# DichenZhang1/libultrahdr_dev

Hardware: AMD Instinct MI355X
Metric: MPixels/sec gain-map generate+apply, 4K P010 batch (higher is better)
Workload: dtype u8/u16 in, f32+f64 math, u8/u32 out

## Files before the change

libultrahdr_dev_amd/csrc/uhdr_kernels.hip:

```cpp
#include "uhdr_kernels.h"

#include <hip/hip_runtime.h>

#include <algorithm>
#include <cmath>

#include "uhdr_apply_px.h"
#include "uhdr_device_math.h"
#include "uhdr_wave_scan.h"

namespace uhdr {

__constant__ float c_idw4[4 * 64];

__constant__ float c_idw4p[64];

hipError_t upload_idw4(const float* tables) {
  float p[64];
  for (int oy = 0; oy < 4; ++oy)
    for (int pr = 0; pr < 2; ++pr)
      for (int k = 0; k < 4; ++k)
        for (int h = 0; h < 2; ++h) p[((oy * 2 + pr) * 4 + k) * 2 + h] = tables[oy * 16 + (2 * pr + h) * 4 + k];
  hipError_t e = hipMemcpyToSymbol(HIP_SYMBOL(c_idw4p), p, sizeof(p));
  if (e != hipSuccess) return e;
  return hipMemcpyToSymbol(HIP_SYMBOL(c_idw4), tables, sizeof(float) * 4 * 64);
}

constexpr float k876 = 1 / 876.0f;
constexpr float k896 = 1 / 896.0f;

constexpr float kP3YR = 0.299f, kP3YG = 0.587f, kP3YB = 0.114f;
constexpr float kP3Cb = 1.772f, kP3Cr = 1.402f;
constexpr float kP3GCb = kP3YB * kP3Cb / kP3YG;
constexpr float kP3GCr = kP3YR * kP3Cr / kP3YG;

typedef float f2 __attribute__((ext_vector_type(2)));
__device__ __forceinline__ f2 pk_fma(f2 a, f2 b, f2 c) { return __builtin_elementwise_fma(a, b, c); }
__device__ __forceinline__ f2 splat(float v) { return (f2){v, v}; }
__device__ __forceinline__ f2 bc_lo(f2 v) { return __builtin_shufflevector(v, v, 0, 0); }
__device__ __forceinline__ f2 bc_hi(f2 v) { return __builtin_shufflevector(v, v, 1, 1); }

__device__ __forceinline__ f2 pk_add_sat(f2 a, f2 b) {
  f2 r;
  asm("v_pk_add_f32 %0, %1, %2 clamp" : "=v"(r) : "v"(a), "v"(b));
  return r;
}
__device__ __forceinline__ f2 pk_mul_sat(f2 a, f2 b) {
  f2 r;
  asm("v_pk_mul_f32 %0, %1, %2 clamp" : "=v"(r) : "v"(a), "v"(b));
  return r;
}
__device__ __forceinline__ f2 pk_fma_sat(f2 a, f2 b, f2 c) {
  f2 r;
  asm("v_pk_fma_f32 %0, %1, %2, %3 clamp" : "=v"(r) : "v"(a), "v"(b), "v"(c));
  return r;
}

template <int HI>
__device__ __forceinline__ f2 pk_fma_sat_bc(f2 a, f2 b, f2 c) {
  f2 r;
  if (HI) asm("v_pk_fma_f32 %0, %1, %2, %3 op_sel:[0,0,1] op_sel_hi:[1,1,1] clamp" : "=v"(r) : "v"(a), "v"(b), "v"(c));
  else asm("v_pk_fma_f32 %0, %1, %2, %3 op_sel_hi:[1,1,0] clamp" : "=v"(r) : "v"(a), "v"(b), "v"(c));
  return r;
}


__device__ __attribute__((noinline)) uint32_t lut_index_wild(float t) {
  const double pos = (double)t + 0.5;
  uint32_t v = 0u;
  if (__builtin_fabs(pos) < 9223372036854775808.0) v = (uint32_t)(long long)pos;
  return v;
}
__device__ __forceinline__ uint32_t round_half_up(float t) {
  int r;
  asm("v_cvt_rpi_i32_f32 %0, %1" : "=v"(r) : "v"(t));
  return (uint32_t)r;
}
__device__ __forceinline__ uint32_t lut_index(float e, uint32_t n) {
  const float t = e * (float)(n - 1u);
  uint32_t v;
  if (__builtin_expect(__float_as_uint(t) < 0x4F000000u, 1)) v = round_half_up(t);
  else v = lut_index_wild(t);
  return min(v, n - 1u);
}
__device__ __forceinline__ uint32_t lut_index_unit(float e, uint32_t n) {
  return round_half_up(e * (float)(n - 1u));
}
__device__ __forceinline__ float gain_lut_entry(uint32_t idx, double log2_min, double log2_max, float boost_factor) {
  const float value = (float)idx / (float)(kGainLutN - 1u);
  const float log_boost = (float)(log2_min * (double)(1.0f - value) + log2_max * (double)value);
  return (float)exp2((double)(log_boost * boost_factor));
}

__global__ void __launch_bounds__(256) k_build_luts(float* lut) {
  const uint32_t i = blockIdx.x * 256u + threadIdx.x;
  if (i >= kLutTotal) return;
  float y;
  if (i < kLutHlgInv) y = srgb_inv_oetf_exact((float)(i - kLutSrgbInv) / (float)(kLutSrgbInvN - 1u));
  else if (i < kLutPqInv) y = hlg_inv_oetf_exact((float)(i - kLutHlgInv) / (float)(kLutHlgInvN - 1u));
  else if (i < kLutHlg) y = pq_inv_oetf_exact((float)(i - kLutPqInv) / (float)(kLutPqInvN - 1u));
  else if (i < kLutPq) y = hlg_oetf_exact((float)(i - kLutHlg) / (float)(kLutHlgN - 1u));
  else y = pq_oetf_exact((float)(i - kLutPq) / (float)(kLutPqN - 1u));
  lut[i] = y;
}
hipError_t launch_build_luts(float* lut, hipStream_t s) {
  hipLaunchKernelGGL(k_build_luts, dim3((kLutTotal + 255u) / 256u), dim3(256), 0, s, lut);
  return hipGetLastError();
}
__global__ void __launch_bounds__(256) k_build_lut_codes(float* lut) {
  const uint32_t i = blockIdx.x * 256u + threadIdx.x;
  const uint32_t t = i >> 16, k = i & 0xFFFFu;
  uint16_t* codes = reinterpret_cast<uint16_t*>(lut + (t ? kCodePq : kCodeHlg));
  codes[k] = (uint16_t)(0x3ffu & (uint32_t)(lut[(t ? kLutPq : kLutHlg) + k] * 1023.0f));
}
hipError_t launch_build_lut_codes(float* lut, hipStream_t s) {
  hipLaunchKernelGGL(k_build_lut_codes, dim3(2u * 65536u / 256u), dim3(256), 0, s, lut);
  return hipGetLastError();
}
__global__ void __launch_bounds__(256) k_build_gain_lut(float* table, double log2_min, double log2_max, float boost_factor) {
  const uint32_t i = blockIdx.x * 256u + threadIdx.x;
  if (i < kGainLutN) table[i] = gain_lut_entry(i, log2_min, log2_max, boost_factor);
}
hipError_t launch_build_gain_lut(float* table, double log2_min, double log2_max, float boost_factor, hipStream_t s) {
  hipLaunchKernelGGL(k_build_gain_lut, dim3(kGainLutN / 256u), dim3(256), 0, s, table, log2_min, log2_max, boost_factor);
  return hipGetLastError();
}


template <int TF>
__device__ __forceinline__ float hdr_inv_oetf(float e) {
  if (TF == 1) return hlg_inv_oetf_guarded(e);
  if (TF == 2) return pq_inv_oetf_guarded(e);
  return e;
}

__device__ __forceinline__ float cvt_word0(uint32_t w) {
  float r;
  asm("v_cvt_f32_u32_sdwa %0, %1 dst_sel:DWORD dst_unused:UNUSED_PAD src0_sel:WORD_0" : "=v"(r) : "v"(w));
  return r;
}
__device__ __forceinline__ float cvt_word1(uint32_t w) {
  float r;
  asm("v_cvt_f32_u32_sdwa %0, %1 dst_sel:DWORD dst_unused:UNUSED_PAD src0_sel:WORD_1" : "=v"(r) : "v"(w));
  return r;
}


constexpr int kGenWhole = 0, kGenFront = 1, kGenBack = 2, kGenLinear = 3, kGenBackLinear = 4;
struct GenMid { f2 r, g, b, hr, hg, hb; };
template <int TF, bool LUT, bool FILTER, bool DEFER = false, int PART = kGenWhole>
__device__ __forceinline__ uint32_t gen_pair(const GenConsts& c, const uint32_t (&hy)[2][4][2],
                                             const uint32_t (&huv)[2][2][2], const uint32_t (&y8)[2][4],
                                             const uint32_t (&u8)[2][2], const uint32_t (&v8)[2][2],
                                             uint8_t (&out)[2], float (&gain)[2], const float* s_srgb, const float* s_hdr,
                                             GenMid* mid = nullptr) {
  f2 r, g, b, hr, hg, hb;
  if (PART == kGenBack || PART == kGenBackLinear) {
    r = mid->r; g = mid->g; b = mid->b; hr = mid->hr; hg = mid->hg; hb = mid->hb;
  } else {
  f2 sy = splat(0.0f), su = splat(0.0f), sv = splat(0.0f);
  f2 hsy = splat(0.0f), hsu = splat(0.0f), hsv = splat(0.0f);
#pragma unroll
  for (int r = 0; r < 2; ++r) {
    f2 uf[2], vf[2], huf[2], hvf[2];
#pragma unroll
    for (int k = 0; k < 2; ++k) {
      const f2 ub = (f2){(float)((u8[0][r] >> (8 * k)) & 0xffu), (float)((u8[1][r] >> (8 * k)) & 0xffu)};
      const f2 vb = (f2){(float)((v8[0][r] >> (8 * k)) & 0xffu), (float)((v8[1][r] >> (8 * k)) & 0xffu)};
      uf[k] = pk_fma(ub, splat(k255), splat(-128.0f * k255));
      vf[k] = pk_fma(vb, splat(k255), splat(-128.0f * k255));
      const uint32_t m0 = huv[0][r][k] & 0xFFC0FFC0u, m1 = huv[1][r][k] & 0xFFC0FFC0u;
      const f2 hu = (f2){cvt_word0(m0), cvt_word0(m1)};
      const f2 hv = (f2){cvt_word1(m0), cvt_word1(m1)};
      huf[k] = pk_fma(hu, splat(k896 * 0.015625f), splat(-64.0f * k896)) - splat(0.5f);
      hvf[k] = pk_fma(hv, splat(k896 * 0.015625f), splat(-64.0f * k896)) - splat(0.5f);
    }
#pragma unroll
    for (int d = 0; d < 2; ++d) {
      const int dy = 2 * r + d;
#pragma unroll
      for (int dx = 0; dx < 4; ++dx) {
        const f2 yb = (f2){(float)((y8[0][dy] >> (8 * dx)) & 0xffu), (float)((y8[1][dy] >> (8 * dx)) & 0xffu)};
        sy += yb * splat(k255);
        su += uf[dx >> 1];
        sv += vf[dx >> 1];
        const uint32_t w0 = hy[0][dy][dx >> 1] & 0xFFC0FFC0u, w1 = hy[1][dy][dx >> 1] & 0xFFC0FFC0u;
        const f2 hb = (dx & 1) ? (f2){cvt_word1(w0), cvt_word1(w1)} : (f2){cvt_word0(w0), cvt_word0(w1)};
        hsy += pk_fma(hb, splat(k876 * 0.015625f), splat(-64.0f * k876));
        hsu += huf[dx >> 1];
        hsv += hvf[dx >> 1];
      }
    }
  }
  sy *= splat(0.0625f); su *= splat(0.0625f); sv *= splat(0.0625f);
  hsy *= splat(0.0625f); hsu *= splat(0.0625f); hsv *= splat(0.0625f);

  r = pk_add_sat(sy, splat(c.sdr_cr) * sv);
  g = pk_add_sat(sy - splat(c.sdr_gcb) * su, -(splat(c.sdr_gcr) * sv));
  b = pk_add_sat(sy, splat(c.sdr_cb) * su);
  hr = pk_add_sat(hsy, splat(c.hdr_cr) * hsv);
  hg = pk_add_sat(hsy - splat(c.hdr_gcb) * hsu, -(splat(c.hdr_gcr) * hsv));
  hb = pk_add_sat(hsy, splat(c.hdr_cb) * hsu);
  }
  static_assert((PART != kGenLinear && PART != kGenBackLinear) || (!LUT && !FILTER), "kGenLinear is the exact path's");
  if (PART != kGenBack && PART != kGenLinear && PART != kGenBackLinear && mid != nullptr) { mid->r = r; mid->g = g; mid->b = b; mid->hr = hr; mid->hg = hg; mid->hb = hb; }
  if (PART == kGenFront) return 0u;

  if (FILTER && !LUT) {
    const f2 fr = (f2){srgb_inv_oetf_fast(r.x), srgb_inv_oetf_fast(r.y)};
    const f2 fg = (f2){srgb_inv_oetf_fast(g.x), srgb_inv_oetf_fast(g.y)};
    const f2 fb = (f2){srgb_inv_oetf_fast(b.x), srgb_inv_oetf_fast(b.y)};
    const f2 fs = (splat(c.lum_r) * fr + splat(c.lum_g) * fg + splat(c.lum_b) * fb) * splat(203.0f);
    f2 qr = hr, qg = hg, qb = hb;
    if (TF == 1) {
      qr = (f2){hlg_inv_oetf_fast(hr.x), hlg_inv_oetf_fast(hr.y)};
      qg = (f2){hlg_inv_oetf_fast(hg.x), hlg_inv_oetf_fast(hg.y)};
      qb = (f2){hlg_inv_oetf_fast(hb.x), hlg_inv_oetf_fast(hb.y)};
    } else if (TF == 2) {
      qr = (f2){pq_inv_oetf_fast(hr.x), pq_inv_oetf_fast(hr.y)};
      qg = (f2){pq_inv_oetf_fast(hg.x), pq_inv_oetf_fast(hg.y)};
      qb = (f2){pq_inv_oetf_fast(hb.x), pq_inv_oetf_fast(hb.y)};
    }
    if (!c.gm_identity) {
      const f2 t0 = splat(c.gm[0]) * qr + splat(c.gm[1]) * qg + splat(c.gm[2]) * qb;
      const f2 t1 = splat(c.gm[3]) * qr + splat(c.gm[4]) * qg + splat(c.gm[5]) * qb;
      const f2 t2 = splat(c.gm[6]) * qr + splat(c.gm[7]) * qg + splat(c.gm[8]) * qb;
      qr = t0; qg = t1; qb = t2;
    }
    const f2 fh = (splat(c.lum_r) * qr + splat(c.lum_g) * qg + splat(c.lum_b) * qb) * splat(c.hdr_white_nits);
    uint32_t fbyte[2], fexact = 0u, doubt = 0u;
    float fgain[2];
#pragma unroll
    for (int k = 0; k < 2; ++k) {
      const float ys = k ? fs.y : fs.x, yh = k ? fh.y : fh.x;
      const float gf = (ys > 0.0f) ? yh * __builtin_amdgcn_rcpf(ys) : 1.0f;
      const float gc = __builtin_amdgcn_fmed3f(gf, c.min_boost, c.max_boost);
      const float v = (__builtin_amdgcn_logf(gc) - c.log2_min) * c.flt_scale;
      const float fl = __builtin_floorf(v), fr2 = v - fl;
      const bool lo = gf < c.flt_lo, hi = gf > c.flt_hi;
      const bool mid = (fr2 >= c.flt_delta) && (fr2 <= 1.0f - c.flt_delta);
      const bool sane = !(ys > 0.0f && ys < 1e-10f) && !(yh != 0.0f && __builtin_fabsf(yh) < 1e-10f);
      if (!((lo || hi || mid) && sane)) doubt |= 1u << k;
      fbyte[k] = lo ? c.enc_byte_min : hi ? c.enc_byte_max : (uint32_t)fl;
      fgain[k] = gf;
      if (!(ys > 0.0f)) fexact |= 1u << k;
    }
    if (DEFER || __builtin_amdgcn_ballot_w64(doubt != 0u) == 0ull) {
      out[0] = (uint8_t)fbyte[0]; out[1] = (uint8_t)fbyte[1];
      gain[0] = fgain[0]; gain[1] = fgain[1];
      return fexact | (doubt << 2);
    }
  }
  constexpr int kLockstep = 6;
  if (LUT) {
    r = (f2){s_srgb[lut_index_unit(r.x, kLutSrgbInvN)], s_srgb[lut_index_unit(r.y, kLutSrgbInvN)]};
    g = (f2){s_srgb[lut_index_unit(g.x, kLutSrgbInvN)], s_srgb[lut_index_unit(g.y, kLutSrgbInvN)]};
    b = (f2){s_srgb[lut_index_unit(b.x, kLutSrgbInvN)], s_srgb[lut_index_unit(b.y, kLutSrgbInvN)]};
  } else {
    float ch[6] = {r.x, r.y, g.x, g.y, b.x, b.y};
#pragma unroll
    for (int i = 0; i < 6; i += kLockstep) {
      float part[kLockstep];
#pragma unroll
      for (int j = 0; j < kLockstep; ++j) part[j] = ch[i + j];
      srgb_inv_oetf_guarded_n<kLockstep>(part);
#pragma unroll
      for (int j = 0; j < kLockstep; ++j) ch[i + j] = part[j];
    }
    r = (f2){ch[0], ch[1]}; g = (f2){ch[2], ch[3]}; b = (f2){ch[4], ch[5]};
  }
  const f2 sdr_nits = (splat(c.lum_r) * r + splat(c.lum_g) * g + splat(c.lum_b) * b) * splat(203.0f);

  if (TF != 0 && LUT) {
    hr = (f2){s_hdr[lut_index_unit(hr.x, kLutHlgInvN)], s_hdr[lut_index_unit(hr.y, kLutHlgInvN)]};
    hg = (f2){s_hdr[lut_index_unit(hg.x, kLutHlgInvN)], s_hdr[lut_index_unit(hg.y, kLutHlgInvN)]};
    hb = (f2){s_hdr[lut_index_unit(hb.x, kLutHlgInvN)], s_hdr[lut_index_unit(hb.y, kLutHlgInvN)]};
  } else if (TF != 0) {
    float ch[6] = {hr.x, hr.y, hg.x, hg.y, hb.x, hb.y};
#pragma unroll
    for (int i = 0; i < 6; i += kLockstep) {
      float part[kLockstep];
#pragma unroll
      for (int j = 0; j < kLockstep; ++j) part[j] = ch[i + j];
      if (TF == 1) hlg_inv_oetf_guarded_n<kLockstep>(part);
      else pq_inv_oetf_guarded_n<kLockstep>(part);
#pragma unroll
      for (int j = 0; j < kLockstep; ++j) ch[i + j] = part[j];
    }
    hr = (f2){ch[0], ch[1]}; hg = (f2){ch[2], ch[3]}; hb = (f2){ch[4], ch[5]};
  }
  if (!c.gm_identity) {
    const f2 t0 = splat(c.gm[0]) * hr + splat(c.gm[1]) * hg + splat(c.gm[2]) * hb;
    const f2 t1 = splat(c.gm[3]) * hr + splat(c.gm[4]) * hg + splat(c.gm[5]) * hb;
    const f2 t2 = splat(c.gm[6]) * hr + splat(c.gm[7]) * hg + splat(c.gm[8]) * hb;
    hr = t0; hg = t1; hb = t2;
  }
  if (PART == kGenLinear || PART == kGenBackLinear) { mid->r = r; mid->g = g; mid->b = b; mid->hr = hr; mid->hg = hg; mid->hb = hb; return 0u; }
  const f2 hdr_nits = (splat(c.lum_r) * hr + splat(c.lum_g) * hg + splat(c.lum_b) * hb) * splat(c.hdr_white_nits);

  gain[0] = raw_gain(sdr_nits.x, hdr_nits.x);
  gain[1] = raw_gain(sdr_nits.y, hdr_nits.y);
#pragma unroll
  for (int k = 0; k < 2; ++k)
    out[k] = encode_gain_guarded(gain[k], c.min_boost, c.max_boost, c.log2_min, c.log2_max, c.enc_scale, c.enc_byte_min,
                                 c.enc_byte_max);
  return 3u;
}

typedef uint32_t u32x4 __attribute__((ext_vector_type(4)));
typedef uint32_t u32x2 __attribute__((ext_vector_type(2)));
__device__ __forceinline__ uint4 ld_stream(const uint4* p) {
  const u32x4 v = __builtin_nontemporal_load(reinterpret_cast<const u32x4*>(p));
  return make_uint4(v.x, v.y, v.z, v.w);
}
__device__ __forceinline__ uint2 ld_stream(const uint2* p) {
  const u32x2 v = __builtin_nontemporal_load(reinterpret_cast<const u32x2*>(p));
  return make_uint2(v.x, v.y);
}
__device__ __forceinline__ uint32_t ld_stream(const uint32_t* p) {
  return __builtin_nontemporal_load(p);
}
__device__ __forceinline__ void st_stream(uint4* p, uint4 v) {
  __builtin_nontemporal_store((u32x4){v.x, v.y, v.z, v.w}, reinterpret_cast<u32x4*>(p));
}
__device__ __forceinline__ void st_stream(uint2* p, uint2 v) {
  __builtin_nontemporal_store((u32x2){v.x, v.y}, reinterpret_cast<u32x2*>(p));
}
__device__ __forceinline__ uint32_t ld8(const uint8_t* p) { return *p; }
__device__ __forceinline__ uint32_t ld16(const uint16_t* p) { return *p; }


template <bool ALIGNED>
__device__ __forceinline__ void load_pair(const GenConsts& c, const GenImage& im, const uint8_t* im_v, uint32_t my, uint32_t pr,
                                          bool two, uint32_t (&hy)[2][4][2], uint32_t (&huv)[2][2][2], uint32_t (&y8)[2][4],
                                          uint32_t (&u8)[2][2], uint32_t (&v8)[2][2]) {
  const uint32_t mx = pr * 2u;
  if (ALIGNED) {
    const uint32_t hoff = 4u * my * im.hy_stride + 8u * pr, yoff = 4u * my * im.y_stride + 8u * pr;
#pragma unroll
    for (int r = 0; r < 4; ++r) {
      const uint4 q = ld_stream(reinterpret_cast<const uint4*>(im.hy + (hoff + r * im.hy_stride)));
      hy[0][r][0] = q.x; hy[0][r][1] = q.y; hy[1][r][0] = q.z; hy[1][r][1] = q.w;
      const uint2 p = ld_stream(reinterpret_cast<const uint2*>(im.y + (yoff + r * im.y_stride)));
      y8[0][r] = p.x; y8[1][r] = p.y;
    }
    const uint32_t huvoff = 2u * my * im.huv_stride + 8u * pr, coff = 2u * my * im.c_stride + 4u * pr;
#pragma unroll
    for (int r = 0; r < 2; ++r) {
      const uint4 q = ld_stream(reinterpret_cast<const uint4*>(im.huv + (huvoff + r * im.huv_stride)));
      huv[0][r][0] = q.x; huv[0][r][1] = q.y; huv[1][r][0] = q.z; huv[1][r][1] = q.w;
      const uint32_t uu = ld_stream(reinterpret_cast<const uint32_t*>(im.u + (coff + r * im.c_stride)));
      const uint32_t vv = ld_stream(reinterpret_cast<const uint32_t*>(im_v + (coff + r * im.c_stride)));
      u8[0][r] = uu & 0xffffu; u8[1][r] = uu >> 16;
      v8[0][r] = vv & 0xffffu; v8[1][r] = vv >> 16;
    }
  } else {
#pragma unroll
    for (int k = 0; k < 2; ++k) {
      const bool on = (k == 0) || two;
      const uint32_t x0 = 4u * (mx + k);
#pragma unroll
      for (int r = 0; r < 4; ++r) {
        const uint16_t* hrow = im.hy + (size_t)(4u * my + r) * im.hy_stride + x0;
        const uint8_t* yrow = im.y + (size_t)(4u * my + r) * im.y_stride + x0;
        hy[k][r][0] = on ? (ld16(hrow) | (ld16(hrow + 1) << 16)) : 0u;
        hy[k][r][1] = on ? (ld16(hrow + 2) | (ld16(hrow + 3) << 16)) : 0u;
        y8[k][r] = on ? (ld8(yrow) | (ld8(yrow + 1) << 8) | (ld8(yrow + 2) << 16) | (ld8(yrow + 3) << 24)) : 0u;
      }
#pragma unroll
      for (int r = 0; r < 2; ++r) {
        const uint16_t* crow = im.huv + (size_t)(2u * my + r) * im.huv_stride + x0;
        const uint8_t* urow = im.u + (size_t)(2u * my + r) * im.c_stride + (x0 >> 1);
        const uint8_t* vrow = im_v + (size_t)(2u * my + r) * im.c_stride + (x0 >> 1);
        huv[k][r][0] = on ? (ld16(crow) | (ld16(crow + 1) << 16)) : 0u;
        huv[k][r][1] = on ? (ld16(crow + 2) | (ld16(crow + 3) << 16)) : 0u;
        u8[k][r] = on ? (ld8(urow) | (ld8(urow + 1) << 8)) : 0u;
        v8[k][r] = on ? (ld8(vrow) | (ld8(vrow + 1) << 8)) : 0u;
      }
    }
  }
}

template <int CTRL, int ROWS>
__device__ __forceinline__ float dpp_move(float v) {
  return __int_as_float(__builtin_amdgcn_update_dpp(__float_as_int(v), __float_as_int(v), CTRL, ROWS, 0xF, false));
}
template <bool MAX>
__device__ __forceinline__ float wave_extreme(float v) {
#define UHDR_EXT(CTRL, ROWS) v = MAX ? fmaxf(v, dpp_move<CTRL, ROWS>(v)) : fminf(v, dpp_move<CTRL, ROWS>(v))
  UHDR_EXT(0xB1, 0xF);
  UHDR_EXT(0x4E, 0xF);
  UHDR_EXT(0x141, 0xF);
  UHDR_EXT(0x140, 0xF);
  UHDR_EXT(0x142, 0xA);
  UHDR_EXT(0x143, 0xC);
#undef UHDR_EXT
  return __int_as_float(__builtin_amdgcn_readlane(__float_as_int(v), 63));
}
__device__ __forceinline__ void wave_minmax(float& vmin, float& vmax) {
  vmin = wave_extreme<false>(vmin);
  vmax = wave_extreme<true>(vmax);
}
__device__ __forceinline__ void publish_minmax(float gmin, float gmax, uint32_t* keys) {
  if ((threadIdx.x & 63u) == 0u && gmin <= gmax) {
    const uint32_t kmin = ~float_to_key(gmin), kmax = float_to_key(gmax);
    if (__hip_atomic_load(&keys[0], __ATOMIC_RELAXED, __HIP_MEMORY_SCOPE_AGENT) < kmin) atomicMax(&keys[0], kmin);
    if (__hip_atomic_load(&keys[1], __ATOMIC_RELAXED, __HIP_MEMORY_SCOPE_AGENT) < kmax) atomicMax(&keys[1], kmax);
  }
}

template <int TF, bool ALIGNED, bool LUT>
__device__ __forceinline__ void exact_pair(const GenConsts& c, const GenImage& im, const uint8_t* im_v, uint32_t my,
                                           uint32_t pr, bool two, const float* s_srgb, const float* s_hdr, uint8_t (&o)[2], float (&gn)[2]) {
  uint32_t hy[2][4][2], huv[2][2][2], y8[2][4], u8[2][2], v8[2][2];
  load_pair<ALIGNED>(c, im, im_v, my, pr, two, hy, huv, y8, u8, v8);
  gen_pair<TF, LUT, false>(c, hy, huv, y8, u8, v8, o, gn, s_srgb, s_hdr);
}


template <int TF, bool ALIGNED, bool LUT, bool FILTER, int TILES, bool DEFER, int BLOCK = kGenBlock>
__global__ void __launch_bounds__(BLOCK, 1) k_generate(const GenConsts c, const GenBatch b) {
  __shared__ float s_srgb[LUT ? kLutSrgbInvN : 1];
  __shared__ float s_hdr[(LUT && TF != 0) ? kLutHlgInvN : 1];
  __shared__ float s_kept[(FILTER && DEFER) ? TILES * 2 * BLOCK : 1];
  if (LUT) {
    for (uint32_t i = threadIdx.x; i < kLutSrgbInvN / 4u; i += BLOCK)
      reinterpret_cast<float4*>(s_srgb)[i] = reinterpret_cast<const float4*>(c.lut + kLutSrgbInv)[i];
    if (TF != 0) {
      const float4* src = reinterpret_cast<const float4*>(c.lut + (TF == 1 ? kLutHlgInv : kLutPqInv));
      for (uint32_t i = threadIdx.x; i < kLutHlgInvN / 4u; i += BLOCK) reinterpret_cast<float4*>(s_hdr)[i] = src[i];
    }
    __syncthreads();
  }
  const uint32_t img_i = blockIdx.x, blk = blockIdx.y;
  const GenImage& im = b.img[img_i];
  const uint8_t* im_v = im.u + (size_t)im.c_stride * (c.height / 2u);
  const uint32_t pairs_per_row = (c.map_w + 1u) >> 1;
  const uint32_t total = pairs_per_row * c.map_h;
  const bool stats = c.stat_keys != nullptr;
  float emin = __builtin_inff(), emax = -__builtin_inff();
  float amin = __builtin_inff(), amax = -__builtin_inff();
  uint32_t kept_exact = 0u, kept_valid = 0u, kept_doubt = 0u;
  uint32_t n_saved = 0u;
  uint32_t* wslot = (FILTER && DEFER && c.stat_slots != 0u)
                        ? c.stat_ws + (size_t)kStatWords * blockIdx.x + kStatHdr + (blockIdx.y * (uint32_t)(BLOCK / 64) + (threadIdx.x >> 6)) * kStatSlotWords
                        : nullptr;

#pragma unroll 1
  for (uint32_t t = 0; t < (uint32_t)TILES; ++t) {
    const uint32_t idx = (blk * (uint32_t)TILES + t) * (uint32_t)BLOCK + threadIdx.x;
    if (idx >= total) break;
    const uint32_t my = idx / pairs_per_row;
    const uint32_t pr = idx - my * pairs_per_row;
    const uint32_t mx = pr * 2u;
    const bool two = ALIGNED || (mx + 1u < c.map_w);

    uint32_t hy[2][4][2], huv[2][2][2], y8[2][4], u8[2][2], v8[2][2];
    load_pair<ALIGNED>(c, im, im_v, my, pr, two, hy, huv, y8, u8, v8);

    uint8_t o[2];
    float gn[2];
    GenMid mid;
    const uint32_t ex = gen_pair<TF, LUT, FILTER, DEFER>(c, hy, huv, y8, u8, v8, o, gn, s_srgb, s_hdr, (FILTER && DEFER) ? &mid : nullptr);
    const uint8_t o0 = o[0], o1 = o[1];
    if (FILTER && DEFER) {
      uint32_t dm = (ex >> 2) & (two ? 3u : 1u);
      if (c.stat_slots != 0u) {
        const unsigned long long dmask = __builtin_amdgcn_ballot_w64(dm != 0u);
        if (dmask != 0ull) {
          const uint32_t pos = n_saved + (uint32_t)__builtin_popcountll(dmask & ((1ull << (threadIdx.x & 63u)) - 1ull));
          n_saved += (uint32_t)__builtin_popcountll(dmask);
          if (dm != 0u && pos < kStatSlotSaved) {
            float4* e = reinterpret_cast<float4*>(wslot + 16u + pos * 16u);
            e[0] = make_float4(__uint_as_float((idx << 3) | dm), mid.r.x, mid.r.y, mid.g.x);
            e[1] = make_float4(mid.g.y, mid.b.x, mid.b.y, mid.hr.x);
            e[2] = make_float4(mid.hr.y, mid.hg.x, mid.hg.y, mid.hb.x);
            e[3] = make_float4(mid.hb.y, 0.0f, 0.0f, 0.0f);
            dm = 0u;
          }
        }
      }
      kept_doubt |= dm << (2u * t);
      if (stats) {
        s_kept[(2u * t) * BLOCK + threadIdx.x] = gn[0];
        s_kept[(2u * t + 1u) * BLOCK + threadIdx.x] = gn[1];
        const uint32_t valid = (two ? 3u : 1u) & ~((ex >> 2) & 3u);
        kept_exact |= (ex & 3u) << (2u * t);
        kept_valid |= valid << (2u * t);
        if (valid & 1u) { amin = fminf(amin, gn[0]); amax = fmaxf(amax, gn[0]); }
        if (valid & 2u) { amin = fminf(amin, gn[1]); amax = fmaxf(amax, gn[1]); }
        if (ex & valid & 1u) { emin = fminf(emin, gn[0]); emax = fmaxf(emax, gn[0]); }
        if (ex & valid & 2u) { emin = fminf(emin, gn[1]); emax = fmaxf(emax, gn[1]); }
      }
    } else {
      emin = fminf(emin, gn[0]); emax = fmaxf(emax, gn[0]);
      if (two) { emin = fminf(emin, gn[1]); emax = fmaxf(emax, gn[1]); }
    }
    uint8_t* mp = im.map + (size_t)my * c.map_w + mx;
    if (ALIGNED) {
      *reinterpret_cast<uint16_t*>(mp) = (uint16_t)(o0 | ((uint32_t)o1 << 8));
    } else {
      mp[0] = o0;
      if (two) mp[1] = o1;
    }
  }
  if (FILTER && !DEFER) return;
  if (!FILTER && !stats) return;
  uint32_t* keys = stats ? c.stat_keys + (size_t)c.stat_stride * img_i : nullptr;

  if (FILTER) {
    uint32_t* ws = c.stat_ws + (size_t)kStatWords * img_i;
    uint32_t cand = 0u;
    if (stats) {
      wave_minmax(amin, amax);
      float wmin = emin, wmax = emax;
      wave_minmax(wmin, wmax);
      const float e = c.flt_gain_rel;
      uint32_t* est = c.stat_spread != 0u ? ws + kStatEst + 2u * (blk % kStatLists) : ws;
      uint32_t e0 = __hip_atomic_load(&est[0], __ATOMIC_RELAXED, __HIP_MEMORY_SCOPE_AGENT);
      uint32_t e1 = __hip_atomic_load(&est[1], __ATOMIC_RELAXED, __HIP_MEMORY_SCOPE_AGENT);
      const uint32_t k0 = __hip_atomic_load(&keys[0], __ATOMIC_RELAXED, __HIP_MEMORY_SCOPE_AGENT);
      const uint32_t k1 = __hip_atomic_load(&keys[1], __ATOMIC_RELAXED, __HIP_MEMORY_SCOPE_AGENT);
      if (amin <= amax) {
        const uint32_t m0 = ~float_to_key(amin), m1 = float_to_key(amax);
        if ((threadIdx.x & 63u) == 0u) {
          if (e0 < m0) atomicMax(&est[0], m0);
          if (e1 < m1) atomicMax(&est[1], m1);
        }
        e0 = e0 < m0 ? m0 : e0; e1 = e1 < m1 ? m1 : e1;
      }
      float min_hi = fminf(k1 != 0u ? key_to_float(~k0) : __builtin_inff(), wmin);
      float max_lo = fmaxf(k1 != 0u ? key_to_float(k1) : -__builtin_inff(), wmax);
      if (e1 != 0u) {
        const float pmin = key_to_float(~e0), pmax = key_to_float(e1);
        min_hi = fminf(min_hi, pmin + e * __builtin_fabsf(pmin));
        max_lo = fmaxf(max_lo, pmax - e * __builtin_fabsf(pmax));
      }
#pragma unroll
      for (uint32_t t = 0; t < (uint32_t)TILES; ++t)
#pragma unroll
        for (uint32_t k = 0; k < 2u; ++k) {
          const uint32_t bit = 1u << (2u * t + k);
          if ((kept_valid & bit) && !(kept_exact & bit)) {
            const float a = s_kept[(2u * t + k) * BLOCK + threadIdx.x], slack = e * __builtin_fabsf(a);
            if ((a - slack <= min_hi) || (a + slack >= max_lo)) cand |= 1u << t;
          }
        }
    }
    unsigned long long mask[TILES];
    uint32_t total = 0u;
#pragma unroll
    for (uint32_t t = 0; t < (uint32_t)TILES; ++t) {
      mask[t] = __builtin_amdgcn_ballot_w64((((kept_doubt >> (2u * t)) & 3u) | ((cand >> t) & 1u)) != 0u);
      total += (uint32_t)__builtin_popcountll(mask[t]);
    }
    if (total != 0u || c.stat_slots != 0u) {
      const uint32_t lane = threadIdx.x & 63u, list = blk % kStatLists;
      uint32_t base = 0u, cap = kStatCap;
      uint32_t* lw = ws + kStatHdr + list * kStatCap;
      if (c.stat_slots != 0u) {
        lw = wslot;
        const bool over = total > kStatSlotPlain;
        const uint32_t ns = n_saved < kStatSlotSaved ? n_saved : kStatSlotSaved;
        if (lane == 0u) {
          ws[kStatSlotCnt + blk * (uint32_t)(BLOCK / 64) + (threadIdx.x >> 6)] = over ? 0u : (total | (ns << 8));
          if (over) __hip_atomic_store(&ws[6], 1u, __ATOMIC_RELAXED, __HIP_MEMORY_SCOPE_AGENT);
        }
        ++lw;
        cap = over ? 0u : kStatSlotPlain;
      } else {
        if (lane == 0u) base = atomicAdd(&ws[8u + list], total);
        base = (uint32_t)__builtin_amdgcn_readfirstlane((int)base);
      }
#pragma unroll
      for (uint32_t t = 0; t < (uint32_t)TILES; ++t) {
        const uint32_t flags = ((kept_doubt >> (2u * t)) & 3u) | (((cand >> t) & 1u) << 2);
        const uint32_t pos = base + (uint32_t)__builtin_popcountll(mask[t] & ((1ull << lane) - 1ull));
        if (flags != 0u && pos < cap) lw[pos] = (((blk * (uint32_t)TILES + t) * (uint32_t)BLOCK + threadIdx.x) << 3) | flags;
        base += (uint32_t)__builtin_popcountll(mask[t]);
      }
    }
    if (!stats) return;
  }
  wave_minmax(emin, emax);
  publish_minmax(emin, emax, keys);
}

__global__ void k_stats_finalize(uint32_t* keys, int n) {
  const int i = blockIdx.x * blockDim.x + threadIdx.x;
  if (i >= n) return;
  const uint32_t k0 = keys[2 * i], k1 = keys[2 * i + 1];
  float mn = __builtin_inff(), mx = -__builtin_inff();
  if (k1 != 0u) { mn = key_to_float(~k0); mx = key_to_float(k1); }
  keys[2 * i] = __float_as_uint(mn);
  keys[2 * i + 1] = __float_as_uint(mx);
}

static_assert(kStatLists == 64u, "k_generate_resolve reads the list counts with one wave");
template <int TF, bool ALIGNED>
__global__ void __launch_bounds__(256) k_generate_resolve(const GenConsts c, const GenBatch b) {
  const uint32_t img_i = blockIdx.x;
  const GenImage& im = b.img[img_i];
  const uint8_t* im_v = im.u + (size_t)im.c_stride * (c.height / 2u);
  uint32_t* ws = c.stat_ws + (size_t)kStatWords * img_i;
  const uint32_t pairs_per_row = (c.map_w + 1u) >> 1, total = pairs_per_row * c.map_h;
  const bool stats = c.stat_out != nullptr;
  float emin = __builtin_inff(), emax = -__builtin_inff();
  __shared__ uint32_t s_first[kStatSlotWaves + 1u];
  __shared__ uint8_t s_ns[kStatSlotWaves];
  __shared__ uint32_t s_sweep;
  const bool slots = c.stat_slots != 0u;
  if (slots) {
    static_assert(kStatSlotWaves == 4u * 256u, "four waves' counts per thread");
    __shared__ uint32_t s_part[4];
    uint32_t n4[4];
    const uint4 cw4 = *reinterpret_cast<const uint4*>(ws + kStatSlotCnt + 4u * threadIdx.x);
    const uint32_t cws[4] = {cw4.x, cw4.y, cw4.z, cw4.w};
#pragma unroll
    for (uint32_t j = 0; j < 4u; ++j) {
      const uint32_t w = 4u * threadIdx.x + j;
      const uint32_t cw = w < c.stat_slots ? cws[j] : 0u;
      s_ns[w] = (uint8_t)(cw >> 8);
      n4[j] = (cw & 0xFFu) + (cw >> 8);
    }
    const uint32_t over = __hip_atomic_load(&ws[6], __ATOMIC_RELAXED, __HIP_MEMORY_SCOPE_AGENT);
    const uint32_t mine = n4[0] + n4[1] + n4[2] + n4[3];
    const uint32_t before = block_exclusive_sum<256>(mine, s_part);
    s_first[4u * threadIdx.x] = before;
    s_first[4u * threadIdx.x + 1u] = before + n4[0];
    s_first[4u * threadIdx.x + 2u] = before + n4[0] + n4[1];
    s_first[4u * threadIdx.x + 3u] = before + n4[0] + n4[1] + n4[2];
    if (threadIdx.x == 255u) { s_first[kStatSlotWaves] = before + mine; s_sweep = over; }
  } else if (threadIdx.x < 64u) {
    const uint32_t cnt = ws[8u + threadIdx.x];
    const bool over = __builtin_amdgcn_ballot_w64(cnt > kStatCap) != 0ull;
    uint32_t inc = min(cnt, kStatCap);
#pragma unroll
    for (int off = 1; off < 64; off <<= 1) {
      const uint32_t v = (uint32_t)__shfl_up((int)inc, off, 64);
      if ((int)threadIdx.x >= off) inc += v;
    }
    s_first[threadIdx.x + 1u] = inc;
    if (threadIdx.x == 0) { s_first[0] = 0u; s_sweep = over ? 1u : 0u; }
  }
  __syncthreads();
  const bool sweep = s_sweep != 0u;
  const uint32_t nl = slots ? kStatSlotWaves : kStatLists;
  const uint32_t n = sweep ? total : s_first[nl];
#pragma unroll 1
  for (uint32_t g = blockIdx.y * 256u + threadIdx.x; g < n; g += kResolveSlices * 256u) {
    uint32_t entry = (g << 3) | 7u;
    GenMid mid;
    bool have = false;
    if (!sweep) {
      uint32_t l = 0u;
      for (uint32_t s2 = nl / 2u; s2 != 0u; s2 >>= 1) if (s_first[l + s2] <= g) l += s2;
      const uint32_t k = g - s_first[l];
      if (!slots) {
        entry = ws[kStatHdr + l * kStatCap + k];
      } else if (k >= (uint32_t)s_ns[l]) {
        entry = ws[kStatHdr + l * kStatSlotWords + 1u + (k - (uint32_t)s_ns[l])];
      } else {
        const uint4* e = reinterpret_cast<const uint4*>(ws + kStatHdr + l * kStatSlotWords + 16u + k * 16u);
        const uint4 e0 = e[0], e1 = e[1], e2 = e[2], e3 = e[3];
        entry = e0.x;
        mid.r = (f2){__uint_as_float(e0.y), __uint_as_float(e0.z)};
        mid.g = (f2){__uint_as_float(e0.w), __uint_as_float(e1.x)};
        mid.b = (f2){__uint_as_float(e1.y), __uint_as_float(e1.z)};
        mid.hr = (f2){__uint_as_float(e1.w), __uint_as_float(e2.x)};
        mid.hg = (f2){__uint_as_float(e2.y), __uint_as_float(e2.z)};
        mid.hb = (f2){__uint_as_float(e2.w), __uint_as_float(e3.x)};
        have = true;
      }
    }
    const uint32_t idx = entry >> 3;
    const uint32_t my = idx / pairs_per_row, pr = idx - my * pairs_per_row;
    const bool two = ALIGNED || (pr * 2u + 1u < c.map_w);
    uint8_t o[2];
    float gn[2];
    uint32_t hy[2][4][2], huv[2][2][2], y8[2][4], u8[2][2], v8[2][2];
    if (!have) {
      load_pair<ALIGNED>(c, im, im_v, my, pr, two, hy, huv, y8, u8, v8);
      gen_pair<TF, false, false, false, kGenFront>(c, hy, huv, y8, u8, v8, o, gn, nullptr, nullptr, &mid);
    }
    gen_pair<TF, false, false, false, kGenBack>(c, hy, huv, y8, u8, v8, o, gn, nullptr, nullptr, &mid);
    uint8_t* mp = im.map + (size_t)my * c.map_w + 2u * pr;
    if (entry & 1u) mp[0] = o[0];
    if ((entry & 2u) && two) mp[1] = o[1];
    if ((entry & 5u) != 0u) { emin = fminf(emin, gn[0]); emax = fmaxf(emax, gn[0]); }
    if ((entry & 6u) != 0u && two) { emin = fminf(emin, gn[1]); emax = fmaxf(emax, gn[1]); }
  }
  if (stats) {
    wave_minmax(emin, emax);
    publish_minmax(emin, emax, ws + 4);
  }
  __shared__ uint32_t s_last;
  asm volatile("s_waitcnt vmcnt(0)" ::: "memory");
  __syncthreads();
  if (threadIdx.x == 0) s_last = atomicAdd(&ws[3], 1u);
  __syncthreads();
  if (s_last == kResolveSlices - 1u && threadIdx.x == 0) {
    if (stats) {
      const uint32_t k0 = __hip_atomic_load(&ws[4], __ATOMIC_RELAXED, __HIP_MEMORY_SCOPE_AGENT);
      const uint32_t k1 = __hip_atomic_load(&ws[5], __ATOMIC_RELAXED, __HIP_MEMORY_SCOPE_AGENT);
      float mn = __builtin_inff(), mx = -__builtin_inff();
      if (k1 != 0u) { mn = key_to_float(~k0); mx = key_to_float(k1); }
      c.stat_out[2u * img_i] = mn;
      c.stat_out[2u * img_i + 1u] = mx;
    }
  }
  __syncthreads();
  static_assert(kStatSlotCnt <= 256u, "one header word per thread");
  if (s_last == kResolveSlices - 1u && threadIdx.x < kStatSlotCnt)
    __hip_atomic_store(&ws[threadIdx.x], 0u, __ATOMIC_RELAXED, __HIP_MEMORY_SCOPE_AGENT);
}
template <int TF>
static hipError_t launch_stats_resolve_tf(const GenConsts& c, const GenBatch& b, int n, bool aligned, hipStream_t s) {
  if (aligned) hipLaunchKernelGGL((k_generate_resolve<TF, true>), dim3((unsigned)n, kResolveSlices), dim3(256), 0, s, c, b);
  else hipLaunchKernelGGL((k_generate_resolve<TF, false>), dim3((unsigned)n, kResolveSlices), dim3(256), 0, s, c, b);
  return hipGetLastError();
}
hipError_t launch_stats_resolve(const GenConsts& c, const GenBatch& b, int n, int hdr_tf, bool aligned, hipStream_t s) {
  if (n <= 0 || c.stat_ws == nullptr) return hipSuccess;
  switch (hdr_tf) {
    case 0: return launch_stats_resolve_tf<0>(c, b, n, aligned, s);
    case 1: return launch_stats_resolve_tf<1>(c, b, n, aligned, s);
    case 2: return launch_stats_resolve_tf<2>(c, b, n, aligned, s);
    default: return hipErrorInvalidValue;
  }
}

bool generate_is_small(const GenConsts& c, int n) {
  const uint32_t total = ((c.map_w + 1u) >> 1) * c.map_h;
  const uint32_t span = (uint32_t)kGenBlock * (uint32_t)kGenTiles;
  return (uint64_t)((total + span - 1u) / span) * (uint64_t)n < 1024u;
}

uint32_t generate_slot_waves(const GenConsts& c, int n) {
// ... 3332 lines not shown
```

Measured before the change: 544,300.

## Tune gain-map generate kernel: packed constant broadcasts, strength-reduced indexing, hoisted loads

Several micro-optimisations in the gain-map generate kernel. Per-image constants are loaded as packed SGPR pairs and broadcast with bc_lo/bc_hi instead of splat. Filter thresholds are moved into VGPRs once per thread. The per-tile division for row/column is replaced by incremental stepping. The log-scale step is done as a packed f2 op. Other changes: shared-memory kept values are loaded unconditionally into registers, and the already-loaded keys are reused to skip reloading atomics in publish_minmax. The aim is fewer scalar-to-vector moves, integer divides and redundant loads, at some cost in register pressure.

```diff
diff --git a/libultrahdr_dev_amd/csrc/uhdr_kernels.hip b/libultrahdr_dev_amd/csrc/uhdr_kernels.hip
--- a/libultrahdr_dev_amd/csrc/uhdr_kernels.hip
+++ b/libultrahdr_dev_amd/csrc/uhdr_kernels.hip
@@ -4,6 +4,7 @@
 
 #include <algorithm>
 #include <cmath>
+#include <cstddef>
 
 #include "uhdr_apply_px.h"
 #include "uhdr_device_math.h"
@@ -147,13 +148,31 @@
 
 
 constexpr int kGenWhole = 0, kGenFront = 1, kGenBack = 2, kGenLinear = 3, kGenBackLinear = 4;
+template <size_t OFFSET>
+__device__ __forceinline__ f2 gen_bcast(const GenConsts& c) {
+  static_assert(OFFSET % 4u == 0u && OFFSET + 4u <= sizeof(GenConsts), "a float of GenConsts");
+  f2 p = *reinterpret_cast<const f2*>(reinterpret_cast<const char*>(&c) + (OFFSET & ~(size_t)7));
+  asm("" : "+s"(p));
+  return (OFFSET & 4u) ? bc_hi(p) : bc_lo(p);
+}
+#define UHDR_BC(c, field) gen_bcast<offsetof(GenConsts, field)>(c)
+struct GenFltRegs { float max_boost, flt_lo, flt_hi, flt_delta, flt_delta1; uint32_t enc_byte_min, enc_byte_max; };
+__device__ __forceinline__ float gen_vgpr(float v) {
+  float r;
+  asm("v_mov_b32 %0, %1" : "=v"(r) : "s"(v));
+  return r;
+}
+__device__ __forceinline__ GenFltRegs gen_flt_in_vgprs(const GenConsts& c) {
+  return {gen_vgpr(c.max_boost), gen_vgpr(c.flt_lo), gen_vgpr(c.flt_hi), gen_vgpr(c.flt_delta), gen_vgpr(1.0f - c.flt_delta),
+          __float_as_uint(gen_vgpr(__uint_as_float(c.enc_byte_min))), __float_as_uint(gen_vgpr(__uint_as_float(c.enc_byte_max)))};
+}
 struct GenMid { f2 r, g, b, hr, hg, hb; };
 template <int TF, bool LUT, bool FILTER, bool DEFER = false, int PART = kGenWhole>
 __device__ __forceinline__ uint32_t gen_pair(const GenConsts& c, const uint32_t (&hy)[2][4][2],
                                              const uint32_t (&huv)[2][2][2], const uint32_t (&y8)[2][4],
                                              const uint32_t (&u8)[2][2], const uint32_t (&v8)[2][2],
                                              uint8_t (&out)[2], float (&gain)[2], const float* s_srgb, const float* s_hdr,
-                                             GenMid* mid = nullptr) {
+                                             GenMid* mid = nullptr, const GenFltRegs* flt = nullptr) {
   f2 r, g, b, hr, hg, hb;
   if (PART == kGenBack || PART == kGenBackLinear) {
     r = mid->r; g = mid->g; b = mid->b; hr = mid->hr; hg = mid->hg; hb = mid->hb;
@@ -195,12 +214,12 @@
   sy *= splat(0.0625f); su *= splat(0.0625f); sv *= splat(0.0625f);
   hsy *= splat(0.0625f); hsu *= splat(0.0625f); hsv *= splat(0.0625f);
 
-  r = pk_add_sat(sy, splat(c.sdr_cr) * sv);
-  g = pk_add_sat(sy - splat(c.sdr_gcb) * su, -(splat(c.sdr_gcr) * sv));
-  b = pk_add_sat(sy, splat(c.sdr_cb) * su);
-  hr = pk_add_sat(hsy, splat(c.hdr_cr) * hsv);
-  hg = pk_add_sat(hsy - splat(c.hdr_gcb) * hsu, -(splat(c.hdr_gcr) * hsv));
-  hb = pk_add_sat(hsy, splat(c.hdr_cb) * hsu);
+  r = pk_add_sat(sy, UHDR_BC(c, sdr_cr) * sv);
+  g = pk_add_sat(sy - UHDR_BC(c, sdr_gcb) * su, -(UHDR_BC(c, sdr_gcr) * sv));
+  b = pk_add_sat(sy, UHDR_BC(c, sdr_cb) * su);
+  hr = pk_add_sat(hsy, UHDR_BC(c, hdr_cr) * hsv);
+  hg = pk_add_sat(hsy - UHDR_BC(c, hdr_gcb) * hsu, -(UHDR_BC(c, hdr_gcr) * hsv));
+  hb = pk_add_sat(hsy, UHDR_BC(c, hdr_cb) * hsu);
   }
   static_assert((PART != kGenLinear && PART != kGenBackLinear) || (!LUT && !FILTER), "kGenLinear is the exact path's");
   if (PART != kGenBack && PART != kGenLinear && PART != kGenBackLinear && mid != nullptr) { mid->r = r; mid->g = g; mid->b = b; mid->hr = hr; mid->hg = hg; mid->hb = hb; }
@@ -210,7 +229,7 @@
     const f2 fr = (f2){srgb_inv_oetf_fast(r.x), srgb_inv_oetf_fast(r.y)};
     const f2 fg = (f2){srgb_inv_oetf_fast(g.x), srgb_inv_oetf_fast(g.y)};
     const f2 fb = (f2){srgb_inv_oetf_fast(b.x), srgb_inv_oetf_fast(b.y)};
-    const f2 fs = (splat(c.lum_r) * fr + splat(c.lum_g) * fg + splat(c.lum_b) * fb) * splat(203.0f);
+    const f2 fs = (UHDR_BC(c, lum_r) * fr + UHDR_BC(c, lum_g) * fg + UHDR_BC(c, lum_b) * fb) * splat(203.0f);
     f2 qr = hr, qg = hg, qb = hb;
     if (TF == 1) {
       qr = (f2){hlg_inv_oetf_fast(hr.x), hlg_inv_oetf_fast(hr.y)};
@@ -222,27 +241,35 @@
       qb = (f2){pq_inv_oetf_fast(hb.x), pq_inv_oetf_fast(hb.y)};
     }
     if (!c.gm_identity) {
-      const f2 t0 = splat(c.gm[0]) * qr + splat(c.gm[1]) * qg + splat(c.gm[2]) * qb;
-      const f2 t1 = splat(c.gm[3]) * qr + splat(c.gm[4]) * qg + splat(c.gm[5]) * qb;
-      const f2 t2 = splat(c.gm[6]) * qr + splat(c.gm[7]) * qg + splat(c.gm[8]) * qb;
+      const f2 t0 = UHDR_BC(c, gm[0]) * qr + UHDR_BC(c, gm[1]) * qg + UHDR_BC(c, gm[2]) * qb;
+      const f2 t1 = UHDR_BC(c, gm[3]) * qr + UHDR_BC(c, gm[4]) * qg + UHDR_BC(c, gm[5]) * qb;
+      const f2 t2 = UHDR_BC(c, gm[6]) * qr + UHDR_BC(c, gm[7]) * qg + UHDR_BC(c, gm[8]) * qb;
       qr = t0; qg = t1; qb = t2;
     }
-    const f2 fh = (splat(c.lum_r) * qr + splat(c.lum_g) * qg + splat(c.lum_b) * qb) * splat(c.hdr_white_nits);
+    const f2 fh = (UHDR_BC(c, lum_r) * qr + UHDR_BC(c, lum_g) * qg + UHDR_BC(c, lum_b) * qb) * UHDR_BC(c, hdr_white_nits);
     uint32_t fbyte[2], fexact = 0u, doubt = 0u;
     float fgain[2];
+    f2 lg;
+    const float max_boost = flt ? flt->max_boost : c.max_boost, flt_lo = flt ? flt->flt_lo : c.flt_lo, flt_hi = flt ? flt->flt_hi : c.flt_hi;
+    const float flt_delta = flt ? flt->flt_delta : c.flt_delta, flt_delta1 = flt ? flt->flt_delta1 : 1.0f - c.flt_delta;
+    const uint32_t enc_byte_min = flt ? flt->enc_byte_min : c.enc_byte_min, enc_byte_max = flt ? flt->enc_byte_max : c.enc_byte_max;
 #pragma unroll
     for (int k = 0; k < 2; ++k) {
       const float ys = k ? fs.y : fs.x, yh = k ? fh.y : fh.x;
-      const float gf = (ys > 0.0f) ? yh * __builtin_amdgcn_rcpf(ys) : 1.0f;
-      const float gc = __builtin_amdgcn_fmed3f(gf, c.min_boost, c.max_boost);
-      const float v = (__builtin_amdgcn_logf(gc) - c.log2_min) * c.flt_scale;
+      fgain[k] = (ys > 0.0f) ? yh * __builtin_amdgcn_rcpf(ys) : 1.0f;
+      lg[k] = __builtin_amdgcn_logf(__builtin_amdgcn_fmed3f(fgain[k], c.min_boost, max_boost));
+    }
+    const f2 v2 = (lg - UHDR_BC(c, log2_min)) * UHDR_BC(c, flt_scale);
+#pragma unroll
+    for (int k = 0; k < 2; ++k) {
+      const float ys = k ? fs.y : fs.x, yh = k ? fh.y : fh.x;
+      const float gf = fgain[k], v = v2[k];
       const float fl = __builtin_floorf(v), fr2 = v - fl;
-      const bool lo = gf < c.flt_lo, hi = gf > c.flt_hi;
-      const bool mid = (fr2 >= c.flt_delta) && (fr2 <= 1.0f - c.flt_delta);
+      const bool lo = gf < flt_lo, hi = gf > flt_hi;
+      const bool mid = (fr2 >= flt_delta) && (fr2 <= flt_delta1);
       const bool sane = !(ys > 0.0f && ys < 1e-10f) && !(yh != 0.0f && __builtin_fabsf(yh) < 1e-10f);
       if (!((lo || hi || mid) && sane)) doubt |= 1u << k;
-      fbyte[k] = lo ? c.enc_byte_min : hi ? c.enc_byte_max : (uint32_t)fl;
-      fgain[k] = gf;
+      fbyte[k] = lo ? enc_byte_min : hi ? enc_byte_max : (uint32_t)fl;
       if (!(ys > 0.0f)) fexact |= 1u << k;
     }
     if (DEFER || __builtin_amdgcn_ballot_w64(doubt != 0u) == 0ull) {
@@ -269,7 +296,7 @@
     }
     r = (f2){ch[0], ch[1]}; g = (f2){ch[2], ch[3]}; b = (f2){ch[4], ch[5]};
   }
-  const f2 sdr_nits = (splat(c.lum_r) * r + splat(c.lum_g) * g + splat(c.lum_b) * b) * splat(203.0f);
+  const f2 sdr_nits = (UHDR_BC(c, lum_r) * r + UHDR_BC(c, lum_g) * g + UHDR_BC(c, lum_b) * b) * splat(203.0f);
 
   if (TF != 0 && LUT) {
     hr = (f2){s_hdr[lut_index_unit(hr.x, kLutHlgInvN)], s_hdr[lut_index_unit(hr.y, kLutHlgInvN)]};
@@ -290,13 +317,13 @@
     hr = (f2){ch[0], ch[1]}; hg = (f2){ch[2], ch[3]}; hb = (f2){ch[4], ch[5]};
   }
   if (!c.gm_identity) {
-    const f2 t0 = splat(c.gm[0]) * hr + splat(c.gm[1]) * hg + splat(c.gm[2]) * hb;
-    const f2 t1 = splat(c.gm[3]) * hr + splat(c.gm[4]) * hg + splat(c.gm[5]) * hb;
-    const f2 t2 = splat(c.gm[6]) * hr + splat(c.gm[7]) * hg + splat(c.gm[8]) * hb;
+    const f2 t0 = UHDR_BC(c, gm[0]) * hr + UHDR_BC(c, gm[1]) * hg + UHDR_BC(c, gm[2]) * hb;
+    const f2 t1 = UHDR_BC(c, gm[3]) * hr + UHDR_BC(c, gm[4]) * hg + UHDR_BC(c, gm[5]) * hb;
+    const f2 t2 = UHDR_BC(c, gm[6]) * hr + UHDR_BC(c, gm[7]) * hg + UHDR_BC(c, gm[8]) * hb;
     hr = t0; hg = t1; hb = t2;
   }
   if (PART == kGenLinear || PART == kGenBackLinear) { mid->r = r; mid->g = g; mid->b = b; mid->hr = hr; mid->hg = hg; mid->hb = hb; return 0u; }
-  const f2 hdr_nits = (splat(c.lum_r) * hr + splat(c.lum_g) * hg + splat(c.lum_b) * hb) * splat(c.hdr_white_nits);
+  const f2 hdr_nits = (UHDR_BC(c, lum_r) * hr + UHDR_BC(c, lum_g) * hg + UHDR_BC(c, lum_b) * hb) * UHDR_BC(c, hdr_white_nits);
 
   gain[0] = raw_gain(sdr_nits.x, hdr_nits.x);
   gain[1] = raw_gain(sdr_nits.y, hdr_nits.y);
@@ -306,6 +333,8 @@
                                  c.enc_byte_max);
   return 3u;
 }
+
+#undef UHDR_BC
 
 typedef uint32_t u32x4 __attribute__((ext_vector_type(4)));
 typedef uint32_t u32x2 __attribute__((ext_vector_type(2)));
@@ -406,6 +435,14 @@
     const uint32_t kmin = ~float_to_key(gmin), kmax = float_to_key(gmax);
     if (__hip_atomic_load(&keys[0], __ATOMIC_RELAXED, __HIP_MEMORY_SCOPE_AGENT) < kmin) atomicMax(&keys[0], kmin);
     if (__hip_atomic_load(&keys[1], __ATOMIC_RELAXED, __HIP_MEMORY_SCOPE_AGENT) < kmax) atomicMax(&keys[1], kmax);
+  }
+}
+
+__device__ __forceinline__ void publish_minmax(float gmin, float gmax, uint32_t* keys, uint32_t k0, uint32_t k1) {
+  if ((threadIdx.x & 63u) == 0u && gmin <= gmax) {
+    const uint32_t kmin = ~float_to_key(gmin), kmax = float_to_key(gmax);
+    if (k0 < kmin) atomicMax(&keys[0], kmin);
+    if (k1 < kmax) atomicMax(&keys[1], kmax);
   }
 }
 
@@ -446,12 +483,19 @@
                         ? c.stat_ws + (size_t)kStatWords * blockIdx.x + kStatHdr + (blockIdx.y * (uint32_t)(BLOCK / 64) + (threadIdx.x >> 6)) * kStatSlotWords
                         : nullptr;
 
+  GenFltRegs flt = {};
+  if (FILTER && DEFER) flt = gen_flt_in_vgprs(c);
+  uint32_t idx = blk * (uint32_t)TILES * (uint32_t)BLOCK + threadIdx.x;
+  uint32_t my = idx / pairs_per_row;
+  uint32_t pr = idx - my * pairs_per_row;
+  uint8_t* map_pair = im.map + 2u * (size_t)idx;
 #pragma unroll 1
-  for (uint32_t t = 0; t < (uint32_t)TILES; ++t) {
-    const uint32_t idx = (blk * (uint32_t)TILES + t) * (uint32_t)BLOCK + threadIdx.x;
+  for (uint32_t t = 0; t < (uint32_t)TILES; ++t, idx += (uint32_t)BLOCK, map_pair += 2 * BLOCK) {
     if (idx >= total) break;
-    const uint32_t my = idx / pairs_per_row;
-    const uint32_t pr = idx - my * pairs_per_row;
+    if (t != 0u) {
+      pr += (uint32_t)BLOCK;
+      while (pr >= pairs_per_row) { pr -= pairs_per_row; ++my; }
+    }
     const uint32_t mx = pr * 2u;
     const bool two = ALIGNED || (mx + 1u < c.map_w);
 
@@ -461,7 +505,8 @@
     uint8_t o[2];
     float gn[2];
     GenMid mid;
-    const uint32_t ex = gen_pair<TF, LUT, FILTER, DEFER>(c, hy, huv, y8, u8, v8, o, gn, s_srgb, s_hdr, (FILTER && DEFER) ? &mid : nullptr);
+    const uint32_t ex = gen_pair<TF, LUT, FILTER, DEFER>(c, hy, huv, y8, u8, v8, o, gn, s_srgb, s_hdr, (FILTER && DEFER) ? &mid : nullptr,
+                                                         (FILTER && DEFER) ? &flt : nullptr);
     const uint8_t o0 = o[0], o1 = o[1];
     if (FILTER && DEFER) {
       uint32_t dm = (ex >> 2) & (two ? 3u : 1u);
@@ -496,10 +541,10 @@
       emin = fminf(emin, gn[0]); emax = fmaxf(emax, gn[0]);
       if (two) { emin = fminf(emin, gn[1]); emax = fmaxf(emax, gn[1]); }
     }
-    uint8_t* mp = im.map + (size_t)my * c.map_w + mx;
     if (ALIGNED) {
-      *reinterpret_cast<uint16_t*>(mp) = (uint16_t)(o0 | ((uint32_t)o1 << 8));
+      *reinterpret_cast<uint16_t*>(map_pair) = (uint16_t)(o0 | ((uint32_t)o1 << 8));
     } else {
+      uint8_t* mp = im.map + (size_t)my * c.map_w + mx;
       mp[0] = o0;
       if (two) mp[1] = o1;
     }
@@ -508,6 +553,7 @@
   if (!FILTER && !stats) return;
   uint32_t* keys = stats ? c.stat_keys + (size_t)c.stat_stride * img_i : nullptr;
 
+  uint32_t k0 = 0u, k1 = 0u;
   if (FILTER) {
     uint32_t* ws = c.stat_ws + (size_t)kStatWords * img_i;
     uint32_t cand = 0u;
@@ -519,8 +565,8 @@
       uint32_t* est = c.stat_spread != 0u ? ws + kStatEst + 2u * (blk % kStatLists) : ws;
       uint32_t e0 = __hip_atomic_load(&est[0], __ATOMIC_RELAXED, __HIP_MEMORY_SCOPE_AGENT);
       uint32_t e1 = __hip_atomic_load(&est[1], __ATOMIC_RELAXED, __HIP_MEMORY_SCOPE_AGENT);
-      const uint32_t k0 = __hip_atomic_load(&keys[0], __ATOMIC_RELAXED, __HIP_MEMORY_SCOPE_AGENT);
-      const uint32_t k1 = __hip_atomic_load(&keys[1], __ATOMIC_RELAXED, __HIP_MEMORY_SCOPE_AGENT);
+      k0 = __hip_atomic_load(&keys[0], __ATOMIC_RELAXED, __HIP_MEMORY_SCOPE_AGENT);
+      k1 = __hip_atomic_load(&keys[1], __ATOMIC_RELAXED, __HIP_MEMORY_SCOPE_AGENT);
       if (amin <= amax) {
         const uint32_t m0 = ~float_to_key(amin), m1 = float_to_key(amax);
         if ((threadIdx.x & 63u) == 0u) {
@@ -536,15 +582,16 @@
         min_hi = fminf(min_hi, pmin + e * __builtin_fabsf(pmin));
         max_lo = fmaxf(max_lo, pmax - e * __builtin_fabsf(pmax));
       }
+      float kept[2 * TILES];
+#pragma unroll
+      for (uint32_t j = 0; j < 2u * (uint32_t)TILES; ++j) kept[j] = s_kept[j * BLOCK + threadIdx.x];
 #pragma unroll
       for (uint32_t t = 0; t < (uint32_t)TILES; ++t)
 #pragma unroll
         for (uint32_t k = 0; k < 2u; ++k) {
           const uint32_t bit = 1u << (2u * t + k);
-          if ((kept_valid & bit) && !(kept_exact & bit)) {
-            const float a = s_kept[(2u * t + k) * BLOCK + threadIdx.x], slack = e * __builtin_fabsf(a);
-            if ((a - slack <= min_hi) || (a + slack >= max_lo)) cand |= 1u << t;
-          }
+          const float a = kept[2u * t + k], slack = e * __builtin_fabsf(a);
+          if ((kept_valid & bit) && !(kept_exact & bit) && ((a - slack <= min_hi) || (a + slack >= max_lo))) cand |= 1u << t;
         }
     }
     unsigned long long mask[TILES];
@@ -583,7 +630,8 @@
     if (!stats) return;
   }
   wave_minmax(emin, emax);
-  publish_minmax(emin, emax, keys);
+  if (FILTER) publish_minmax(emin, emax, keys, k0, k1);
+  else publish_minmax(emin, emax, keys);
 }
 
 __global__ void k_stats_finalize(uint32_t* keys, int n) {
```

Result: no change. 546,200 (median of 6 runs) (+0.4%).
